# jdfxzzy/DPMN

Measured on AMD Instinct MI355X. Metric: SR images/sec (16x64->32x128, bs=48 per GPU, fp32 forward), higher is better.
Workload: dtype f32; 1 GPU; cfg1: TATT PSN + 3+3 PGRM (embed 96, windows 2/4/8) + CMM, forward-only; per_gpu_batch=48, global_batch=48, ranks=1, batches_in_flight=2, parallelism=dp1 (independent batch shards, no forward collective)

## Files before the change

### dpmn_amd/_abi.py

```python
import ctypes as C
import os

import torch

_HERE = os.path.dirname(os.path.abspath(__file__))
LIB_PATH = os.environ.get("DPMN_HIP_LIB") or os.path.join(_HERE, "lib", "libdpmn_hip.so")

if not os.path.exists(LIB_PATH):
    raise RuntimeError(
        "dpmn_amd: %s not found -- build it with `python -c 'import __graft_entry__ as g; g.build()'` "
        "(or `make -C dpmn_amd/csrc`).  There is no CPU fallback for the DPMN hot path." % LIB_PATH)

lib = C.CDLL(LIB_PATH)

fp = C.c_void_p


class PgrmBlock(C.Structure):
    _fields_ = [(n, fp) for n in (
        "norm1_q_w", "norm1_q_b", "norm1_kv_w", "norm1_kv_b", "q_w", "q_b", "kv_w", "kv_b")] + [
        ("bias_table", fp * 4)] + [(n, fp) for n in (
            "sk_proj_w", "sk_proj_b", "sk_fc1_w", "sk_fc1_b", "sk_fc2_w", "sk_fc2_b", "sk_head_w", "sk_head_b",
            "norm2_w", "norm2_b", "fc1_w", "fc1_b", "dw_w", "dw_b", "pw_w", "pw_b", "fc2_w", "fc2_b")]

# ... 118 lines not shown
    "dpmn_distill_forward_f32": (_i, [C.POINTER(DistillParams), fp, fp, _i, fp, fp, fp, fp, fp, _sz, _i, _i, _i, fp]),
    "dpmn_distill_backward_f32": (_i, [C.POINTER(DistillParams), C.POINTER(DistillGrads), fp, fp, fp, fp, fp, fp, fp, fp, fp, _sz, _i, _i, _i, fp]),
    "dpmn_conv2d_wgrad_unpack_multi_f32": (_i, [fp, fp, _i, _i, fp]),
    "dpmn_tl_interp_f32": (_i, [fp, fp, _i, _i, _i, _i, _i, fp]),
    "dpmn_pointwise_wgrad_det_bytes": (_sz, [_i, _i]),
    "dpmn_reduce_defer_begin": (_i, []),
    "dpmn_reduce_defer_enable": (_i, [_i]),
    "dpmn_reduce_defer_push": (_i, [C.POINTER(TnPending)]),
    "dpmn_reduce_defer_pending": (_i, []),
    "dpmn_reduce_defer_flush": (_i, [_i, fp]),
    "dpmn_xred_fallbacks": (_i, [C.POINTER(C.c_uint), _i]),
    "dpmn_selftest_xshfl": (_i, [C.POINTER(C.c_uint)]),
    "dpmn_selftest_lds_poison": (_i, [C.c_uint, _i, fp]),
    "dpmn_xred_test_force_recompute": (_i, [_i]),
    "dpmn_xred_enable": (_i, [_i]),
    "dpmn_nchw_to_nhwc_f32": (_i, [fp, fp, _i, _i, _i, _i, _i, fp]),
    "dpmn_nhwc_to_nchw_f32": (_i, [fp, fp, _i, _i, _i, _i, fp]),
    "dpmn_se_gate_f32": (_i, [fp, fp, fp, fp, fp, fp, fp, _i, _i, _i, _i, fp]),
    "dpmn_bigru_f32": (_i, [fp, fp, fp, fp, fp, _i, _i, _i, C.c_long, C.c_long, C.c_long, _i, fp]),
    "dpmn_small_linear_f32": (_i, [fp, fp, _i, fp, fp, fp, _i, _i, _i, _i, _f, fp]),
    "dpmn_tatt_encoder_layer_f32": (_i, [fp, fp, _PP, fp, _i, _i, _i, _i, fp]),
    "dpmn_cross_attn_f32": (_i, [fp, fp, fp, fp, fp, _i, _i, _i, _i, _i, fp]),
    "dpmn_add_layernorm64_f32": (_i, [fp, fp, fp, fp, fp, fp, fp, fp, _f, _i, C.c_long, fp]),
    "dpmn_gru_gate_f32": (_i, [fp, fp, fp, fp, C.c_long, _i, _i, fp]),
    "dpmn_to_mask_f32": (_i, [fp, C.c_long, fp, _i, _i, _i, fp]),
    "dpmn_mha32_f32": (_i, [fp, fp, _i, _i, _i, _f, fp]),
    "dpmn_layernorm_std_f32": (_i, [fp, fp, fp, _f, fp, _l, _i, fp]),
    "dpmn_rotate_img_f32": (_i, [fp, fp, fp, _f, fp, _i, _i, _i, _i, fp]),
    "dpmn_blend_f32": (_i, [fp, C.c_long, fp, C.c_long, fp, _f, _i, _i, fp]),
    "dpmn_psnr_ssim_workspace_bytes": (_sz, [_i, _i, _i, _i]),
# ... 227 lines not shown
```

### dpmn_amd/csrc/conv.hip

```cpp
#include "conv_body.h"

namespace {

template <int BM, int BN, int WM, int WN, bool UNI = false, bool SIMPLE = false, bool AFF = false, bool BF = false>
__global__ __launch_bounds__(256) void k_conv_igemm(ConvArgs a) {
  conv_igemm_body<BM, BN, WM, WN, UNI, SIMPLE, AFF, BF>(a);
}
template <int BM, int BN, int WM, int WN, bool AFF>
__global__ __launch_bounds__(256, 2) void k_conv_igemm_xr(ConvArgs a) {
  conv_igemm_body<BM, BN, WM, WN, true, true, AFF, false, true>(a);
}

__global__ __launch_bounds__(256) void k_conv_splitk_reduce(ConvArgs a, int rows, int cq_lanes) {
  __shared__ float red[256][8];
  const PhaseSel ph = conv_select_phase(a, blockIdx.z * a.ksplit);
  const int M = a.B * a.Hp * a.Wp;
  const int n4 = a.npad / 4;
  const int cl = threadIdx.x & (cq_lanes - 1), rl = threadIdx.x / cq_lanes, RL = 256 / cq_lanes;
  const int cq = blockIdx.x * cq_lanes + cl;
  const int n = cq * 4;
  const int m_lo = blockIdx.y * rows;
  float ssum[4] = {0.f, 0.f, 0.f, 0.f}, ssq[4] = {0.f, 0.f, 0.f, 0.f};
  const size_t zs = (size_t)M * a.npad;
  if (cq < n4) {
// ... 704 lines not shown
  for (int i = 0; i < 3; ++i)
    uni = uni && a.cseg[i] % 32 == 0 && (size_t)a.B * a.Hin * a.Win * a.cseg[i] * 4 < (1ull << 31);
  {
    ProfScope prof(BN == 128 ? PT_CONV_IGEMM_128 : (BN == 64 ? PT_CONV_IGEMM_64 : PT_CONV_IGEMM_NARROW), st, conv_flops(a), conv_bytes(a));
    static const int xred_env = getenv("DPMN_CONV_XRED") ? atoi(getenv("DPMN_CONV_XRED")) : 0;
    const int xred_on = g_xred_enabled >= 0 ? g_xred_enabled : xred_env;
    bool simple = uni && a.KH * a.KW <= 31 && (a.pro_act == ACT_NONE || a.pro_act == ACT_RELU || a.pro_act == ACT_LEAKY02);
    int n_seg = 0, n_aff = 0;
    for (int i = 0; i < 3; ++i) {
      if (a.cseg[i] > 0) { ++n_seg; n_aff += a.in_scale[i] != nullptr; }
      simple = simple &&
               ((size_t)a.B * a.Hin * a.Win + (size_t)(abs(a.pad_y) + a.KH * abs(a.dil_y) + 2) * a.Win) * a.cseg[i] * 4 < (1ull << 31);
    }
    simple = simple && (n_aff == 0 || n_aff == n_seg);
  if (g_dpmn_x3 && simple && BM == 128 && BN == 128) {
    if (dpmn_conv::x3_launch_igemm(n_aff != 0, a, grid, st) != 0) return dpmn_set_error(DPMN_ERR_LAUNCH, "conv2d: bf16x3 launch failed");
  } else
  if (g_dpmn_bf16 && simple && BM == BN && (BM == 128 || BM == 64)) {
    if (n_aff) hipLaunchKernelGGL((k_conv_igemm<BM, BN, WM, WN, true, true, true, true>), grid, dim3(256), 0, st, a);
    else hipLaunchKernelGGL((k_conv_igemm<BM, BN, WM, WN, true, true, false, true>), grid, dim3(256), 0, st, a);
  } else
  if (simple && S > 1 && BM == 128 && BN == 128 && xred_on && cnt && xred_fits(tiles, S, cnt_len, a) &&
           (size_t)tiles * S * BM * BN * sizeof(float) <= ws_bytes) {
    if constexpr (BM == 128 && BN == 128) {
      const int tm = cdiv(M, BM), tn = cdiv(a.Cout, BN), t8 = cdiv(tiles, 8);
      double cost[2];
      for (int order = 0; order < 2; ++order) {
        double wsets = 0, xsets = 0;
        for (int c = 0; c < 8; ++c) {
          const int t0 = c * t8, t1 = (c + 1) * t8 < tiles ? (c + 1) * t8 : tiles;
          if (t0 >= t1) break;
// ... 9 lines not shown
          }
        }
        cost[order] = wsets * BN * (double)a.Kp + xsets * BM * (double)a.stride * a.stride * a.cin;
      }
      static const int force_order = getenv("DPMN_XRED_ORDER") ? atoi(getenv("DPMN_XRED_ORDER")) : -1;
      static const int ablate = getenv("DPMN_XRED_ABLATE") ? atoi(getenv("DPMN_XRED_ABLATE")) : 0;
      a.xr_cnt = cnt; a.xr_tm = tm; a.xr_tn = tn; a.xr_t8 = t8; a.xr_force_redo = g_xred_force_recompute; a.xr_ablate = ablate;
      a.xr_order = force_order >= 0 ? force_order : (cost[0] <= cost[1] ? 0 : 1);
      a.wlocal = 0;
      const dim3 g1(8 * t8 * S);
      if (n_aff) hipLaunchKernelGGL((k_conv_igemm_xr<BM, BN, WM, WN, true>), g1, dim3(256), 0, st, a);
      else hipLaunchKernelGGL((k_conv_igemm_xr<BM, BN, WM, WN, false>), g1, dim3(256), 0, st, a);
      DPMN_CHECK_LAUNCH();
      return DPMN_OK;
    }
  }
  else if (simple && n_aff) hipLaunchKernelGGL((k_conv_igemm<BM, BN, WM, WN, true, true, true>), grid, dim3(256), 0, st, a);
  else if (simple) hipLaunchKernelGGL((k_conv_igemm<BM, BN, WM, WN, true, true>), grid, dim3(256), 0, st, a);
  else if (uni) hipLaunchKernelGGL((k_conv_igemm<BM, BN, WM, WN, true>), grid, dim3(256), 0, st, a);
    else hipLaunchKernelGGL((k_conv_igemm<BM, BN, WM, WN>), grid, dim3(256), 0, st, a);
  }
  DPMN_CHECK_LAUNCH();
  if (S > 1) {
    ProfScope prof(PT_CONV_SPLITK_REDUCE, st, 0.0, 4.0 * (double)(S + 1) * nph * M * a.npad);
    const int n4 = a.npad / 4;
    const int cql = n4 >= 64 ? 64 : (n4 >= 32 ? 32 : 16);
    const int cb = cdiv(n4, cql);
    int rows = cb * cdiv(M, 64) >= 1024 ? 64 : (cb * cdiv(M, 16) >= 1024 ? 16 : 4);
    if (rows < 256 / cql) rows = 256 / cql;
    hipLaunchKernelGGL(k_conv_splitk_reduce, dim3(cb, cdiv(M, rows), nph), dim3(256), 0, st, a, rows, cql);
// ... 115 lines not shown
  unsigned v = 0;
  if (hipMemcpyFromSymbol(&v, HIP_SYMBOL(g_xred_fallbacks), sizeof(v)) != hipSuccess) return dpmn_set_error(DPMN_ERR_RUNTIME, "xred_fallbacks: copy failed");
  *count_out = v;
  if (reset) {
    v = 0;
    if (hipMemcpyToSymbol(HIP_SYMBOL(g_xred_fallbacks), &v, sizeof(v)) != hipSuccess) return dpmn_set_error(DPMN_ERR_RUNTIME, "xred_fallbacks: reset failed");
  }
  return DPMN_OK;
}

int dpmn_xred_enable(int on) {
  g_xred_enabled = on < 0 ? -1 : (on ? 1 : 0);
  return DPMN_OK;
}

int dpmn_xred_test_force_recompute(int on) {
  g_xred_force_recompute = on ? 1 : 0;
  return DPMN_OK;
}

int dpmn_nchw_to_nhwc_f32(const float* in, float* out, int B, int C, int H, int W, int Cpad, dpmn_stream_t stream) {
  DPMN_REQUIRE(in && out && Cpad >= C, "nchw_to_nhwc: bad arguments");
  const long total = (long)B * H * W;
  hipLaunchKernelGGL(k_nchw_to_nhwc, dim3((unsigned)((total + 255) / 256)), dim3(256), 0, as_stream(stream), in, out, B, C, H, W, Cpad);
  DPMN_CHECK_LAUNCH();
  return DPMN_OK;
}

int dpmn_nhwc_to_nchw_f32(const float* in, float* out, int B, int C, int H, int W, dpmn_stream_t stream) {
  DPMN_REQUIRE(in && out, "nhwc_to_nchw: bad arguments");
// ... 8 lines not shown
```

### dpmn_amd/csrc/conv_body.h

```cpp
#pragma once
#include <cstdlib>
#include <type_traits>
#include "common.h"

namespace dpmn_conv {
struct ConvArgs {
  const float* in[3];
  const float* in_scale[3];
  const float* in_shift[3];
  int cseg[3];
  int cin;
  int B, Hin, Win;
  int KH, KW, stride, dil_y, dil_x, pad_y, pad_x;
  int Hp, Wp;
  int Hout, Wout, ostep, ooy, oox;
  int pro_act;
  const float* w;
  int Kp;
  const float* bias;
  int Cout;
  int epi_act;
  float slope;
  const float* res;
  float* out;
// ... 6 lines not shown
  int npad;
  int nphase;
  long wps;
  int groups;
  int m_per_group;
  long wgs;
  int wlocal;
  unsigned* xr_cnt;
  int xr_tm, xr_tn;
  int xr_t8;
  int xr_order;
  int xr_force_redo;
  int xr_group;
  int xr_cstride;
  int xr_ablate;
};
int x3_launch_igemm(bool aff, const ConvArgs& a, dim3 grid, hipStream_t st);
int x3_launch_halo(const ConvArgs& a, dim3 grid, hipStream_t st);
}

namespace {

constexpr int PAD = 4, BK = 32, LDK = BK + PAD;
constexpr int STAT_SLOTS = 32;

using dpmn_conv::ConvArgs;
int g_xred_enabled = -1;
int g_xred_force_recompute = 0;
__device__ unsigned g_xred_fallbacks = 0;
__device__ __forceinline__ int conv_group_of(const ConvArgs& a, int m) { return (a.groups > 1 && m >= a.m_per_group) ? 1 : 0; }

struct PhaseSel {
// ... 57 lines not shown
        if (n + r < a.Cout) {
          const float t = v[r] + (a.res ? a.res[o + r] : 0.f);
          a.out[o + r] = post ? fmaxf(t, 0.f) : t;
        }
    }
  }
}

__device__ __forceinline__ float vmax_raw(float x, float y) {
  float r;
  asm("v_max_f32 %0, %1, %2" : "=v"(r) : "v"(x), "v"(y));
  return r;
}

template <int BM, int BN, int WM, int WN, bool UNI = false, bool SIMPLE = false, bool AFF = false, bool BF = false, bool XRED = false,
          bool X3 = false>
__device__ __forceinline__ void conv_igemm_body(const ConvArgs& a) {
  static_assert(!X3 || (SIMPLE && !BF && !XRED), "the bf16x3 variant exists for the SIMPLE path");
  static_assert(!XRED || SIMPLE, "the in-L2 reduction exists for the SIMPLE path");
  static_assert(!BF || SIMPLE, "the bf16 variant exists for the SIMPLE path");
  static_assert(!SIMPLE || UNI, "SIMPLE is a refinement of the UNI path");
  static_assert(!AFF || SIMPLE, "AFF is a variant of the SIMPLE path");
  constexpr int MT = BM / WM / 16, NT = BN / WN / 16;
  constexpr int TPR = BK / 4, RPP = 256 / TPR;
  constexpr int APASS = BM / RPP, BPASS = (BN + RPP - 1) / RPP;
  constexpr int LDKB = X3 ? BK + 16 : BK + 8;
  constexpr bool B16 = BF || X3;
  constexpr int NPL = X3 ? 3 : 1;
  constexpr int NBUF = X3 ? 1 : 2;
  constexpr int XPL = BM * LDKB, WPL = BN * LDKB;
  typedef typename std::conditional<B16, unsigned short, float>::type lds_t;
  __shared__ __attribute__((aligned(16))) lds_t Xs[NBUF][NPL * BM * (B16 ? LDKB : LDK)];
// ... 1 lines not shown

  const int tid = threadIdx.x, lane = tid & 63, wave = tid >> 6;
  const int M = a.B * a.Hp * a.Wp;
  int bx = blockIdx.x, by = blockIdx.y, bz = blockIdx.z;
  int xr_tile = 0;
  if constexpr (XRED) {
    const int L = blockIdx.x, c = L & 7, j = L >> 3;
    const int tl = j / a.ksplit, z = j - tl * a.ksplit;
    const int nph_ = a.nphase > 1 ? a.nphase : 1;
    xr_tile = c * a.xr_t8 + tl;
    if (tl >= a.xr_t8 || xr_tile >= a.xr_tm * a.xr_tn * nph_) return;
    int phs;
    if (a.xr_order == 0) { bx = xr_tile % a.xr_tm; const int r = xr_tile / a.xr_tm; by = r % a.xr_tn; phs = r / a.xr_tn; }
    else { by = xr_tile % a.xr_tn; const int r = xr_tile / a.xr_tn; phs = r % nph_; bx = r / nph_; }
    bz = phs * a.ksplit + z;
  } else
  if (a.wlocal) {
    const int L = bx + gridDim.x * (by + gridDim.y * bz);
    const int c = L & 7, j = L >> 3;
    const int jm = j / (int)gridDim.x;
    bx = j - jm * (int)gridDim.x;
    const int nz = c + 8 * jm;
    by = nz / (int)gridDim.z;
    bz = nz - by * (int)gridDim.z;
  }
  const int m_blk = bx * BM, n_blk = by * BN;
  const PhaseSel ph = conv_select_phase(a, bz, m_blk);
  const int zsplit = ph.zsplit;
  const int lrow = tid / TPR, lcol = (tid % TPR) * 4;

  int pb[APASS], py[APASS], px[APASS];
  const int HWp = a.Hp * a.Wp;
  const float inv_hw = 1.0f / (float)HWp, inv_w = 1.0f / (float)a.Wp;
#pragma unroll
  for (int p = 0; p < APASS; ++p) {
    const int m = m_blk + lrow + p * RPP;
    if (m < M) {
      int b = (int)((float)m * inv_hw), r = m - b * HWp;
      if (r < 0) { --b; r += HWp; }
      if (r >= HWp) { ++b; r -= HWp; }
      int y = (int)((float)r * inv_w), x = r - y * a.Wp;
      if (x < 0) { --y; x += a.Wp; }
      if (x >= a.Wp) { ++y; x -= a.Wp; }
      pb[p] = b;
      py[p] = y * a.stride - ph.pad_y;
      px[p] = x * a.stride - ph.pad_x;
    } else {
      pb[p] = -1; py[p] = 0; px[p] = 0;
    }
  }
  const int c01 = a.cseg[0] + a.cseg[1];
  const int ktaps = a.KH * a.KW;

  float4 xr[APASS], wr[BPASS];
  float4 s4r, h4r;
  unsigned vmask = 0;
  bool has_aff = false;
  auto gload = [&](int k0) {
    const int k = k0 + lcol;
    const int tap = k / a.cin, c = k - tap * a.cin;
    const int ky = tap / a.KW, kx = tap - ky * a.KW;
    const int dy = ky * a.dil_y, dx = kx * a.dil_x;
    int seg = 0, cl = c;
    if (c >= c01) { seg = 2; cl = c - c01; }
    else if (c >= a.cseg[0]) { seg = 1; cl = c - a.cseg[0]; }
// ... 10 lines not shown
      const int iy = py[p] + dy, ix = px[p] + dx;
      const bool ok = pb[p] >= 0 && tap_ok && iy >= 0 && iy < a.Hin && ix >= 0 && ix < a.Win;
      xr[p] = ok ? *reinterpret_cast<const float4*>(src + (((size_t)pb[p] * a.Hin + iy) * a.Win + ix) * cs + cl)
                 : make_float4(0.f, 0.f, 0.f, 0.f);
      vmask |= (ok ? 1u : 0u) << p;
    }
#pragma unroll
    for (int p = 0; p < BPASS; ++p) {
      const int r = lrow + p * RPP;
      const int n = n_blk + r;
      wr[p] = (r < BN && n < a.Cout) ? *reinterpret_cast<const float4*>(ph.w + (size_t)n * a.Kp + k0 + lcol)
                                     : make_float4(0.f, 0.f, 0.f, 0.f);
    }
  };
  typedef int i32x4_ __attribute__((ext_vector_type(4)));
  int pix[APASS];
#pragma unroll
  for (int p = 0; p < APASS; ++p) {
    pix[p] = pb[p] >= 0 ? (pb[p] * a.Hin + py[p]) * a.Win + px[p] : 0;
    if (pb[p] < 0) { py[p] = -(1 << 20); px[p] = -(1 << 20); }
  }
  int u_tap = 0, u_c0 = 0, u_ky = 0, u_kx = 0, u_k0 = -2;
  int wofs[BPASS];
#pragma unroll
  for (int p = 0; p < BPASS; ++p) wofs[p] = ((n_blk + lrow + p * RPP) * a.Kp + lcol) * 4;
  auto gload_uni = [&](int k0) {
    if (k0 == u_k0 + BK) {
      u_c0 += BK;
      if (u_c0 >= a.cin) { u_c0 = 0; ++u_tap; if (++u_kx == a.KW) { u_kx = 0; ++u_ky; } }
    } else if (k0 != u_k0) {
      u_tap = k0 / a.cin; u_c0 = k0 - u_tap * a.cin;
      u_ky = u_tap / a.KW; u_kx = u_tap - u_ky * a.KW;
    }
    u_k0 = k0;
    const int tap = u_tap, c0 = u_c0, ky = u_ky, kx = u_kx;
    const bool tap_ok = tap < ktaps;
    const int dy = tap_ok ? ky * a.dil_y : (1 << 21), dx = kx * a.dil_x;
    const int seg = c0 >= c01 ? 2 : (c0 >= a.cseg[0] ? 1 : 0);
    const int cl = c0 - (seg == 2 ? c01 : (seg == 1 ? a.cseg[0] : 0)) + lcol;
    const float* src = a.in[seg];
// ... 8 lines not shown
    vmask = 0;
#pragma unroll
    for (int p = 0; p < APASS; ++p) {
      const bool ok = (unsigned)(py[p] + dy) < (unsigned)a.Hin && (unsigned)(px[p] + dx) < (unsigned)a.Win;
      const unsigned off = (unsigned)((__mul24(pix[p] + tapoff, cs) + cl) * 4) | (ok ? 0u : 0x80000000u);
      xr[p] = __builtin_bit_cast(float4, __builtin_amdgcn_raw_buffer_load_b128(xrs, (int)off, 0, 0));
      vmask |= (ok ? 1u : 0u) << p;
    }
#pragma unroll
    for (int p = 0; p < BPASS; ++p) {
      const int r = lrow + p * RPP;
      if (BN % RPP == 0 || r < BN)
        wr[p] = __builtin_bit_cast(float4, __builtin_amdgcn_raw_buffer_load_b128(wrs, wofs[p], k0 * 4, 0));
    }
  };
  unsigned nok[APASS];
  int voff[APASS];
  int s_seg = -1, s_segstart = 0;
  __amdgpu_buffer_rsrc_t s_xrs, s_scrs, s_shrs;
  unsigned inv[APASS];
  const int padoff = ph.pad_y * a.Win + ph.pad_x;
  const int minoff = (a.dil_y < 0 ? (a.KH - 1) * a.dil_y : 0) * a.Win + (a.dil_x < 0 ? (a.KW - 1) * a.dil_x : 0);
  const int baseshift = padoff - minoff;
  if (SIMPLE) {
#pragma unroll
    for (int p = 0; p < APASS; ++p) {
      unsigned colm = 0, okb = 0;
      for (int kx = 0; kx < a.KW; ++kx) colm |= ((unsigned)(px[p] + kx * a.dil_x) < (unsigned)a.Win ? 1u : 0u) << kx;
      for (int ky = 0; ky < a.KH; ++ky)
        if ((unsigned)(py[p] + ky * a.dil_y) < (unsigned)a.Hin) okb |= colm << (ky * a.KW);
      nok[p] = ~okb;
    }
  }
  const __amdgpu_buffer_rsrc_t s_wrs = __builtin_amdgcn_make_buffer_rsrc(const_cast<float*>(ph.w), 0, a.Cout * a.Kp * 4, 0x00020000);
  auto gload_simple = [&](int kt_) {
    if (kt_ == u_k0 + 1) {
      ++u_tap;
      if (++u_kx == a.KW) { u_kx = 0; ++u_ky; }
      if (u_tap == ktaps) { u_tap = 0; u_ky = 0; u_c0 += BK; }
    } else if (kt_ != u_k0) {
      const int cch = kt_ / ktaps;
      u_tap = kt_ - cch * ktaps; u_c0 = cch * BK;
      u_ky = u_tap / a.KW; u_kx = u_tap - u_ky * a.KW;
    }
    u_k0 = kt_;
    const int k0 = u_tap * a.cin + u_c0;
    const int seg = u_c0 >= c01 ? 2 : (u_c0 >= a.cseg[0] ? 1 : 0);
    const int cs = seg == 2 ? a.cseg[2] : (seg == 1 ? a.cseg[1] : a.cseg[0]);
    if (seg != s_seg) {
// ... 99 lines not shown
      } else if ((vmask >> p) & 1u) {
        if (has_aff) { v.x = v.x * s4r.x + h4r.x; v.y = v.y * s4r.y + h4r.y; v.z = v.z * s4r.z + h4r.z; v.w = v.w * s4r.w + h4r.w; }
        if (a.pro_act != ACT_NONE) {
          v.x = apply_act(v.x, a.pro_act, 0.f); v.y = apply_act(v.y, a.pro_act, 0.f);
          v.z = apply_act(v.z, a.pro_act, 0.f); v.w = apply_act(v.w, a.pro_act, 0.f);
        }
      }
      *reinterpret_cast<float4*>(&Xs[buf][(lrow + p * RPP) * LDK + lcol]) = v;
    }
#pragma unroll
    for (int p = 0; p < BPASS; ++p)
      if (lrow + p * RPP < BN) *reinterpret_cast<float4*>(&Ws[buf][(lrow + p * RPP) * LDK + lcol]) = wr[p];
    }
  };

  const int wm = wave % WM, wn = wave / WM;
  const int lr = lane & 15, kq = lane >> 4;
  f32x4 acc[NT][MT];
#pragma unroll
  for (int i = 0; i < NT; ++i)
#pragma unroll
    for (int j = 0; j < MT; ++j) acc[i][j] = (f32x4){0.f, 0.f, 0.f, 0.f};

  const int nk_all = a.Kp / BK;
  const int cps = (nk_all + a.ksplit - 1) / a.ksplit;
  int zcur = zsplit;
  int mode = 0;
  for (;;) {
  const int kt0 = zcur * cps;
  const int nk = min(nk_all, kt0 + cps);
  if constexpr (XRED) {
#pragma unroll
    for (int i = 0; i < NT; ++i)
#pragma unroll
      for (int j = 0; j < MT; ++j) acc[i][j] = (f32x4){0.f, 0.f, 0.f, 0.f};
  }
  if (kt0 < nk) {
    if (SIMPLE) { gload_simple(kt0); sstore_simple(0); }
    else {
      if (UNI) gload_uni(kt0 * BK); else gload(kt0 * BK);
      sstore(0);
    }
  }
  __syncthreads();
  for (int kt = kt0; kt < nk; ++kt) {
    const int buf = NBUF == 2 ? (kt - kt0) & 1 : 0;
    if (SIMPLE) gload_simple(min(kt + 1, nk - 1));
    else if (UNI) gload_uni(min(kt + 1, nk - 1) * BK);
    else if (kt + 1 < nk) gload((kt + 1) * BK);
    if (UNI) __builtin_amdgcn_sched_barrier(0);
    if constexpr (X3) {
      const lds_t* xa = &Xs[buf][(wm * (MT * 16) + lr) * LDKB + kq * 8];
      const lds_t* wa = &Ws[buf][(wn * (NT * 16) + lr) * LDKB + kq * 8];
      bf16x8 w0[NT], w1[NT], w2[NT], xp[MT], xq[MT];
#pragma unroll
      for (int i = 0; i < NT; ++i) {
        w0[i] = *reinterpret_cast<const bf16x8*>(wa + i * 16 * LDKB);
// ... 36 lines not shown
#pragma unroll
      for (int i = 0; i < NT; ++i) wf[i] = *reinterpret_cast<const f32x4*>(wa + i * 16 * LDK + kc);
#pragma unroll
      for (int s = 0; s < 4; ++s)
#pragma unroll
        for (int i = 0; i < NT; ++i)
#pragma unroll
          for (int j = 0; j < MT; ++j) acc[i][j] = mfma16(wf[i][s], xf[j][s], acc[i][j]);
    }
    }
    if (NBUF == 1) __syncthreads();
    if (SIMPLE) sstore_simple(NBUF == 2 ? buf ^ 1 : 0);
    else if (UNI || kt + 1 < nk) sstore(buf ^ 1);
    __syncthreads();
  }
  if constexpr (!XRED) break;
  else {
    if (a.ksplit <= 1) break;
    constexpr int QN = NT * MT, HQ = QN / 2;
    static_assert(QN % 2 == 0, "the collect moves half slots");
    typedef int i32x4x_ __attribute__((ext_vector_type(4)));
    const int S = a.ksplit, GS = a.xr_group, ngrp = (S + GS - 1) / GS;
    const int g_lo = (zsplit / GS) * GS, g_hi = min(S, g_lo + GS);
    const __amdgpu_buffer_rsrc_t prs = __builtin_amdgcn_make_buffer_rsrc(a.partial, 0, a.xr_tm * a.xr_tn * (a.nphase > 1 ? a.nphase : 1) * S * (QN * 4096), 0x00020000);
    constexpr int SC1 = 0x10;
    auto slot_of = [&](int z_) { return __builtin_amdgcn_readfirstlane((xr_tile * S + z_) * (QN * 4096)); };
    auto st_slot = [&](int z_) {
      const int so = slot_of(z_);
#pragma unroll
      for (int i = 0; i < NT; ++i)
#pragma unroll
// ... 78 lines not shown
        break;
      }
    }
    if (to_l2) {
      if (ngrp == 1) break;
      st_slot(g_lo);
      const int f = arrive(words + ngrp * a.xr_cstride, ngrp);
      if (f == 0) return;
      if (f == 2) { mode = 2; zcur = 0; continue; }
      if (!(a.xr_ablate & 1)) collect(0, ngrp, GS);
    }
    break;
  }
  }

  if (!XRED && a.ksplit > 1) {
#pragma unroll
    for (int j = 0; j < MT; ++j) {
      const int m = m_blk + wm * (MT * 16) + j * 16 + lr;
      if (m >= M) continue;
#pragma unroll
      for (int i = 0; i < NT; ++i) {
        const int n = n_blk + wn * (NT * 16) + i * 16 + kq * 4;
        if (n >= a.npad) continue;
        *reinterpret_cast<float4*>(ph.partial + ((size_t)zsplit * M + m) * a.npad + n) =
            make_float4(acc[i][j][0], acc[i][j][1], acc[i][j][2], acc[i][j][3]);
      }
    }
    return;
  }
  float ssum[NT][4], ssq[NT][4];
#pragma unroll
  for (int i = 0; i < NT; ++i)
#pragma unroll
    for (int r = 0; r < 4; ++r) { ssum[i][r] = 0.f; ssq[i][r] = 0.f; }
#pragma unroll
  for (int j = 0; j < MT; ++j) {
    const int m = m_blk + wm * (MT * 16) + j * 16 + lr;
    if (m >= M) continue;
#pragma unroll
    for (int i = 0; i < NT; ++i) {
      const int n = n_blk + wn * (NT * 16) + i * 16 + kq * 4;
      if (n >= a.Cout) continue;
      float v[4] = {acc[i][j][0], acc[i][j][1], acc[i][j][2], acc[i][j][3]};
      conv_store(a, m, n, v, ssum[i], ssq[i], ph.ooy, ph.oox);
    }
  }
  if (a.stats) {
#pragma unroll
    for (int i = 0; i < NT; ++i) {
      const int n = n_blk + wn * (NT * 16) + i * 16 + kq * 4;
#pragma unroll
      for (int r = 0; r < 4; ++r) {
        float s = ssum[i][r], q = ssq[i][r];
        s += xshfl<1>(s); s += xshfl<2>(s); s += xshfl<4>(s); s += xshfl<8>(s);
        q += xshfl<1>(q); q += xshfl<2>(q); q += xshfl<4>(q); q += xshfl<8>(q);
        if (lr == 0 && n + r < a.Cout) {
          double* st = reinterpret_cast<double*>(a.stats) + (size_t)(bx % STAT_SLOTS) * 2 * a.Cout;
          atomicAdd(st + n + r, (double)(s));
          atomicAdd(st + a.Cout + n + r, (double)(q));
        }
      }
    }
  }
}

template <int KS, int BN, int TH, bool BF = false, bool X3 = false>
__device__ __forceinline__ void conv_halo_body(const ConvArgs& a) {
  static_assert(!(BF && X3), "one operand format");
  constexpr int NTH = 256, RPS = NTH / 8;
  constexpr int LDH = (BF || X3) ? (BK + 8) / 2 : LDK;
  constexpr int NPL = X3 ? 3 : 1;
  constexpr int TW = 16, HH = TH + KS - 1, HW_ = TW + KS - 1, NPX = HH * HW_;
  constexpr int NT = BN / 16, T = KS * KS, MR = TH / 4;
  constexpr int WV = (BN * 8 + NTH - 1) / NTH;
  constexpr int TPS = 1;
  extern __shared__ __attribute__((aligned(16))) float smem[];
  float* halo = smem;
  float* Wt = smem + NPL * NPX * LDH;
// ... 267 lines not shown
```

### dpmn_amd/csrc/conv_x3.hip

```cpp
#include "conv_body.h"

namespace {
template <int BM, int BN, int WM, int WN, bool AFF>
__global__ __launch_bounds__(256, 2) void k_conv_igemm_x3(ConvArgs a) {
  conv_igemm_body<BM, BN, WM, WN, true, true, AFF, false, false, true>(a);
}
}

namespace dpmn_conv {
int x3_launch_igemm(bool aff, const ConvArgs& a, dim3 grid, hipStream_t st) {
  if (aff) hipLaunchKernelGGL((k_conv_igemm_x3<128, 128, 2, 2, true>), grid, dim3(256), 0, st, a);
  else hipLaunchKernelGGL((k_conv_igemm_x3<128, 128, 2, 2, false>), grid, dim3(256), 0, st, a);
  return 0;
}
int x3_launch_halo(const ConvArgs& a, dim3 grid, hipStream_t st) {
  constexpr int NPX = (8 + 2) * (16 + 2);
  const size_t smem = (size_t)(3 * NPX + 2 * 3 * 64) * ((BK + 8) / 2) * sizeof(float);
  static bool attr_set = false;
  if (!attr_set) {
    (void)hipFuncSetAttribute(reinterpret_cast<const void*>(&k_conv_halo_x3<3, 64, 8>), hipFuncAttributeMaxDynamicSharedMemorySize, (int)smem);
    attr_set = true;
  }
  hipLaunchKernelGGL((k_conv_halo_x3<3, 64, 8>), grid, dim3(256), smem, st, a);
  return 0;
}
}
```

### include/dpmn_hip.h

```cpp
#ifndef DPMN_HIP_H
#define DPMN_HIP_H

#include <stddef.h>
#include <stdint.h>

#ifdef __cplusplus
extern "C" {
#endif

typedef void* dpmn_stream_t;

enum { DPMN_OK = 0, DPMN_ERR_ARG = -1, DPMN_ERR_LAUNCH = -2, DPMN_ERR_WORKSPACE = -3, DPMN_ERR_RUNTIME = -4 };

enum { DPMN_ACT_NONE = 0, DPMN_ACT_GELU = 1, DPMN_ACT_RELU = 2, DPMN_ACT_LEAKY02 = 3, DPMN_ACT_LEAKY001 = 4,
       DPMN_ACT_MISH = 5, DPMN_ACT_PRELU = 6, DPMN_ACT_TANH = 7, DPMN_ACT_SIGMOID = 8,
       DPMN_ACT_RELU_POST_RES = 9  };

int dpmn_abi_version(void);
const char* dpmn_last_error(void);
int dpmn_set_compute_dtype(int mode);
int dpmn_get_compute_dtype(void);

int dpmn_linear_f32(const float* x, const float* w, const float* bias, const float* res1, const float* res2,
                    float* y, int M, int N, int K, int act, float slope, dpmn_stream_t stream);
// ... 84 lines not shown
  float* stats;
  float* splitk_ws;
  size_t splitk_ws_bytes;
  int nphase;
  long w_phase_stride;
  int groups;
  long w_group_stride;
  unsigned* arrive_cnt;
  int arrive_cnt_len;
} dpmn_conv_desc;
int dpmn_conv2d_nhwc_f32(const dpmn_conv_desc* d, dpmn_stream_t stream);
int dpmn_xred_fallbacks(unsigned* count_out, int reset);
int dpmn_selftest_xshfl(unsigned* mismatches_out);
int dpmn_selftest_lds_poison(unsigned pattern, int blocks, dpmn_stream_t stream);
int dpmn_xred_enable(int on);
int dpmn_xred_test_force_recompute(int on);
int dpmn_nchw_to_nhwc_f32(const float* in, float* out, int B, int C, int H, int W, int Cpad, dpmn_stream_t stream);
int dpmn_nhwc_to_nchw_f32(const float* in, float* out, int B, int C, int H, int W, dpmn_stream_t stream);

typedef struct {
  const float *conv_cat_w, *conv_cat_b;
  const float *bn1_w, *bn1_b;
  float *bn1_rm, *bn1_rv;
  long long* bn1_nbt;
  const float *conv_feat_w, *conv_feat_b;
  const float *bn2_w, *bn2_b;
  float *bn2_rm, *bn2_rv;
  long long* bn2_nbt;
} dpmn_distill_params;
typedef struct {
// ... 394 lines not shown
```

Baseline: 6319 images/s.

## Make implicit-GEMM conv kernels persistent with next-tile prefetch overlapping epilogue

Turns the square-tile implicit-GEMM conv kernels, including the bf16x3 variant, into persistent kernels. Each launch sizes its grid to device capacity (CU count times occupancy), and every block loops over output tiles. Before running the current tile's epilogue, a block decodes the next tile and issues its first global fetch, so loads overlap the stores. This is meant to cut wave-tail and launch-granularity costs on small conv grids, at the price of extra register pressure, changed launch bounds, and serialized tiles when there are fewer units than capacity.

New measurement: 6342 images/s (median of 6 runs). No clear change (+0.4%).

```diff
diff --git a/dpmn_amd/_abi.py b/dpmn_amd/_abi.py
--- a/dpmn_amd/_abi.py
+++ b/dpmn_amd/_abi.py
@@ -156,6 +156,7 @@
     "dpmn_selftest_lds_poison": (_i, [C.c_uint, _i, fp]),
     "dpmn_xred_test_force_recompute": (_i, [_i]),
     "dpmn_xred_enable": (_i, [_i]),
+    "dpmn_conv_persist_blocks": (_i, [_i]),
     "dpmn_nchw_to_nhwc_f32": (_i, [fp, fp, _i, _i, _i, _i, _i, fp]),
     "dpmn_nhwc_to_nchw_f32": (_i, [fp, fp, _i, _i, _i, _i, fp]),
     "dpmn_se_gate_f32": (_i, [fp, fp, fp, fp, fp, fp, fp, _i, _i, _i, _i, fp]),
diff --git a/dpmn_amd/csrc/conv.hip b/dpmn_amd/csrc/conv.hip
--- a/dpmn_amd/csrc/conv.hip
+++ b/dpmn_amd/csrc/conv.hip
@@ -6,6 +6,11 @@
 __global__ __launch_bounds__(256) void k_conv_igemm(ConvArgs a) {
   conv_igemm_body<BM, BN, WM, WN, UNI, SIMPLE, AFF, BF>(a);
 }
+template <int BM, int BN, int WM, int WN, bool UNI = false, bool SIMPLE = false, bool AFF = false>
+__global__ __launch_bounds__(256, BM == 64 ? 4 : 2) void k_conv_igemm_p(ConvArgs a) {
+  conv_igemm_body<BM, BN, WM, WN, UNI, SIMPLE, AFF, false, false, false, true>(a);
+}
+int g_persist_blocks = 0;
 template <int BM, int BN, int WM, int WN, bool AFF>
 __global__ __launch_bounds__(256, 2) void k_conv_igemm_xr(ConvArgs a) {
   conv_igemm_body<BM, BN, WM, WN, true, true, AFF, false, true>(a);
@@ -742,7 +747,7 @@
     }
     simple = simple && (n_aff == 0 || n_aff == n_seg);
   if (g_dpmn_x3 && simple && BM == 128 && BN == 128) {
-    if (dpmn_conv::x3_launch_igemm(n_aff != 0, a, grid, st) != 0) return dpmn_set_error(DPMN_ERR_LAUNCH, "conv2d: bf16x3 launch failed");
+    if (dpmn_conv::x3_launch_igemm(n_aff != 0, a, grid, g_persist_blocks, st) != 0) return dpmn_set_error(DPMN_ERR_LAUNCH, "conv2d: bf16x3 launch failed");
   } else
   if (g_dpmn_bf16 && simple && BM == BN && (BM == 128 || BM == 64)) {
     if (n_aff) hipLaunchKernelGGL((k_conv_igemm<BM, BN, WM, WN, true, true, true, true>), grid, dim3(256), 0, st, a);
@@ -782,6 +787,12 @@
       DPMN_CHECK_LAUNCH();
       return DPMN_OK;
     }
+  }
+  else if constexpr (BM == BN) {
+    if (simple && n_aff) launch_conv_units<k_conv_igemm_p<BM, BN, WM, WN, true, true, true>>(a, grid, g_persist_blocks, st);
+    else if (simple) launch_conv_units<k_conv_igemm_p<BM, BN, WM, WN, true, true>>(a, grid, g_persist_blocks, st);
+    else if (uni) launch_conv_units<k_conv_igemm_p<BM, BN, WM, WN, true>>(a, grid, g_persist_blocks, st);
+    else launch_conv_units<k_conv_igemm_p<BM, BN, WM, WN>>(a, grid, g_persist_blocks, st);
   }
   else if (simple && n_aff) hipLaunchKernelGGL((k_conv_igemm<BM, BN, WM, WN, true, true, true>), grid, dim3(256), 0, st, a);
   else if (simple) hipLaunchKernelGGL((k_conv_igemm<BM, BN, WM, WN, true, true>), grid, dim3(256), 0, st, a);
@@ -927,6 +938,12 @@
   return DPMN_OK;
 }
 
+int dpmn_conv_persist_blocks(int n) {
+  const int old = g_persist_blocks;
+  g_persist_blocks = n < 0 ? -1 : n;
+  return old;
+}
+
 int dpmn_xred_test_force_recompute(int on) {
   g_xred_force_recompute = on ? 1 : 0;
   return DPMN_OK;
diff --git a/dpmn_amd/csrc/conv_body.h b/dpmn_amd/csrc/conv_body.h
--- a/dpmn_amd/csrc/conv_body.h
+++ b/dpmn_amd/csrc/conv_body.h
@@ -44,8 +44,10 @@
   int xr_group;
   int xr_cstride;
   int xr_ablate;
+  int p_units;
+  int p_gx, p_gy, p_gz;
 };
-int x3_launch_igemm(bool aff, const ConvArgs& a, dim3 grid, hipStream_t st);
+int x3_launch_igemm(bool aff, const ConvArgs& a, dim3 grid, int blocks, hipStream_t st);
 int x3_launch_halo(const ConvArgs& a, dim3 grid, hipStream_t st);
 }
 
@@ -133,8 +135,9 @@
 }
 
 template <int BM, int BN, int WM, int WN, bool UNI = false, bool SIMPLE = false, bool AFF = false, bool BF = false, bool XRED = false,
-          bool X3 = false>
+          bool X3 = false, bool PERSIST = false>
 __device__ __forceinline__ void conv_igemm_body(const ConvArgs& a) {
+  static_assert(!PERSIST || !XRED, "the in-L2 reduction keeps its own block-to-tile map");
   static_assert(!X3 || (SIMPLE && !BF && !XRED), "the bf16x3 variant exists for the SIMPLE path");
   static_assert(!XRED || SIMPLE, "the in-L2 reduction exists for the SIMPLE path");
   static_assert(!BF || SIMPLE, "the bf16 variant exists for the SIMPLE path");
@@ -166,41 +169,95 @@
     if (a.xr_order == 0) { bx = xr_tile % a.xr_tm; const int r = xr_tile / a.xr_tm; by = r % a.xr_tn; phs = r / a.xr_tn; }
     else { by = xr_tile % a.xr_tn; const int r = xr_tile / a.xr_tn; phs = r % nph_; bx = r / nph_; }
     bz = phs * a.ksplit + z;
-  } else
-  if (a.wlocal) {
-    const int L = bx + gridDim.x * (by + gridDim.y * bz);
-    const int c = L & 7, j = L >> 3;
-    const int jm = j / (int)gridDim.x;
-    bx = j - jm * (int)gridDim.x;
-    const int nz = c + 8 * jm;
-    by = nz / (int)gridDim.z;
-    bz = nz - by * (int)gridDim.z;
-  }
-  const int m_blk = bx * BM, n_blk = by * BN;
-  const PhaseSel ph = conv_select_phase(a, bz, m_blk);
-  const int zsplit = ph.zsplit;
-  const int lrow = tid / TPR, lcol = (tid % TPR) * 4;
-
+  }
+  int m_blk = 0, n_blk = 0, zsplit = 0;
+  PhaseSel ph{};
+  const int lrow0 = tid / TPR, lcol0 = (tid % TPR) * 4;
+  const int lrow = lrow0, lcol = lcol0;
   int pb[APASS], py[APASS], px[APASS];
   const int HWp = a.Hp * a.Wp;
   const float inv_hw = 1.0f / (float)HWp, inv_w = 1.0f / (float)a.Wp;
-#pragma unroll
-  for (int p = 0; p < APASS; ++p) {
-    const int m = m_blk + lrow + p * RPP;
-    if (m < M) {
-      int b = (int)((float)m * inv_hw), r = m - b * HWp;
-      if (r < 0) { --b; r += HWp; }
-      if (r >= HWp) { ++b; r -= HWp; }
-      int y = (int)((float)r * inv_w), x = r - y * a.Wp;
-      if (x < 0) { --y; x += a.Wp; }
-      if (x >= a.Wp) { ++y; x -= a.Wp; }
-      pb[p] = b;
-      py[p] = y * a.stride - ph.pad_y;
-      px[p] = x * a.stride - ph.pad_x;
-    } else {
-      pb[p] = -1; py[p] = 0; px[p] = 0;
-    }
-  }
+  int pix[APASS];
+  int u_tap = 0, u_c0 = 0, u_ky = 0, u_kx = 0, u_k0 = -2;
+  int wofs[BPASS];
+  unsigned nok[APASS];
+  int s_seg = -1;
+  int padoff = 0, baseshift = 0;
+  const int minoff = (a.dil_y < 0 ? (a.KH - 1) * a.dil_y : 0) * a.Win + (a.dil_x < 0 ? (a.KW - 1) * a.dil_x : 0);
+  __amdgpu_buffer_rsrc_t s_wrs;
+  auto unit_decode = [&](int L) {
+    int lrow = lrow0, lcol = lcol0;
+    if constexpr (PERSIST) {
+      asm volatile("" : "+v"(lrow), "+v"(lcol));
+      const int gx = a.p_gx, gy = a.p_gy, gz = a.p_gz;
+      if (a.wlocal) {
+        const int c = L & 7, j = L >> 3;
+        const int jm = j / gx;
+        bx = j - jm * gx;
+        const int nz = c + 8 * jm;
+        by = nz / gz;
+        bz = nz - by * gz;
+      } else {
+        const int r = L / gx;
+        bx = L - r * gx;
+        bz = r / gy;
+        by = r - bz * gy;
+      }
+    } else if constexpr (!XRED) {
+      if (a.wlocal) {
+        const int L_ = bx + gridDim.x * (by + gridDim.y * bz);
+        const int c = L_ & 7, j = L_ >> 3;
+        const int jm = j / (int)gridDim.x;
+        bx = j - jm * (int)gridDim.x;
+        const int nz = c + 8 * jm;
+        by = nz / (int)gridDim.z;
+        bz = nz - by * (int)gridDim.z;
+      }
+    }
+    m_blk = bx * BM; n_blk = by * BN;
+    ph = conv_select_phase(a, bz, m_blk);
+    zsplit = ph.zsplit;
+#pragma unroll
+    for (int p = 0; p < APASS; ++p) {
+      const int m = m_blk + lrow + p * RPP;
+      if (m < M) {
+        int b = (int)((float)m * inv_hw), r = m - b * HWp;
+        if (r < 0) { --b; r += HWp; }
+        if (r >= HWp) { ++b; r -= HWp; }
+        int y = (int)((float)r * inv_w), x = r - y * a.Wp;
+        if (x < 0) { --y; x += a.Wp; }
+        if (x >= a.Wp) { ++y; x -= a.Wp; }
+        pb[p] = b;
+        py[p] = y * a.stride - ph.pad_y;
+        px[p] = x * a.stride - ph.pad_x;
+      } else {
+        pb[p] = -1; py[p] = 0; px[p] = 0;
+      }
+    }
+#pragma unroll
+    for (int p = 0; p < APASS; ++p) {
+      pix[p] = pb[p] >= 0 ? (pb[p] * a.Hin + py[p]) * a.Win + px[p] : 0;
+      if (pb[p] < 0) { py[p] = -(1 << 20); px[p] = -(1 << 20); }
+    }
+    u_k0 = -2; s_seg = -1;
+#pragma unroll
+    for (int p = 0; p < BPASS; ++p) wofs[p] = ((n_blk + lrow + p * RPP) * a.Kp + lcol) * 4;
+    padoff = ph.pad_y * a.Win + ph.pad_x;
+    baseshift = padoff - minoff;
+    if (SIMPLE) {
+#pragma unroll
+      for (int p = 0; p < APASS; ++p) {
+        unsigned colm = 0, okb = 0;
+        for (int kx = 0; kx < a.KW; ++kx) colm |= ((unsigned)(px[p] + kx * a.dil_x) < (unsigned)a.Win ? 1u : 0u) << kx;
+        for (int ky = 0; ky < a.KH; ++ky)
+          if ((unsigned)(py[p] + ky * a.dil_y) < (unsigned)a.Hin) okb |= colm << (ky * a.KW);
+        nok[p] = ~okb;
+      }
+    }
+    s_wrs = __builtin_amdgcn_make_buffer_rsrc(const_cast<float*>(ph.w), 0, a.Cout * a.Kp * 4, 0x00020000);
+  };
+  int unit = PERSIST ? (int)blockIdx.x : 0;
+  unit_decode(unit);
   const int c01 = a.cseg[0] + a.cseg[1];
   const int ktaps = a.KH * a.KW;
 
@@ -241,16 +298,6 @@
     }
   };
   typedef int i32x4_ __attribute__((ext_vector_type(4)));
-  int pix[APASS];
-#pragma unroll
-  for (int p = 0; p < APASS; ++p) {
-    pix[p] = pb[p] >= 0 ? (pb[p] * a.Hin + py[p]) * a.Win + px[p] : 0;
-    if (pb[p] < 0) { py[p] = -(1 << 20); px[p] = -(1 << 20); }
-  }
-  int u_tap = 0, u_c0 = 0, u_ky = 0, u_kx = 0, u_k0 = -2;
-  int wofs[BPASS];
-#pragma unroll
-  for (int p = 0; p < BPASS; ++p) wofs[p] = ((n_blk + lrow + p * RPP) * a.Kp + lcol) * 4;
   auto gload_uni = [&](int k0) {
     if (k0 == u_k0 + BK) {
       u_c0 += BK;
@@ -289,25 +336,10 @@
         wr[p] = __builtin_bit_cast(float4, __builtin_amdgcn_raw_buffer_load_b128(wrs, wofs[p], k0 * 4, 0));
     }
   };
-  unsigned nok[APASS];
   int voff[APASS];
-  int s_seg = -1, s_segstart = 0;
+  int s_segstart = 0;
   __amdgpu_buffer_rsrc_t s_xrs, s_scrs, s_shrs;
   unsigned inv[APASS];
-  const int padoff = ph.pad_y * a.Win + ph.pad_x;
-  const int minoff = (a.dil_y < 0 ? (a.KH - 1) * a.dil_y : 0) * a.Win + (a.dil_x < 0 ? (a.KW - 1) * a.dil_x : 0);
-  const int baseshift = padoff - minoff;
-  if (SIMPLE) {
-#pragma unroll
-    for (int p = 0; p < APASS; ++p) {
-      unsigned colm = 0, okb = 0;
-      for (int kx = 0; kx < a.KW; ++kx) colm |= ((unsigned)(px[p] + kx * a.dil_x) < (unsigned)a.Win ? 1u : 0u) << kx;
-      for (int ky = 0; ky < a.KH; ++ky)
-        if ((unsigned)(py[p] + ky * a.dil_y) < (unsigned)a.Hin) okb |= colm << (ky * a.KW);
-      nok[p] = ~okb;
-    }
-  }
-  const __amdgpu_buffer_rsrc_t s_wrs = __builtin_amdgcn_make_buffer_rsrc(const_cast<float*>(ph.w), 0, a.Cout * a.Kp * 4, 0x00020000);
   auto gload_simple = [&](int kt_) {
     if (kt_ == u_k0 + 1) {
       ++u_tap;
@@ -437,8 +469,9 @@
     }
   };
 
-  const int wm = wave % WM, wn = wave / WM;
-  const int lr = lane & 15, kq = lane >> 4;
+  const int wm0 = wave % WM, wn0 = wave / WM;
+  const int lr0 = lane & 15, kq0 = lane >> 4;
+  const int wm = wm0, wn = wn0, lr = lr0, kq = kq0;
   f32x4 acc[NT][MT];
 #pragma unroll
   for (int i = 0; i < NT; ++i)
@@ -449,6 +482,68 @@
   const int cps = (nk_all + a.ksplit - 1) / a.ksplit;
   int zcur = zsplit;
   int mode = 0;
+  auto first_fetch = [&](int z_) {
+    const int k_ = z_ * cps;
+    if (k_ < nk_all) {
+      if (SIMPLE) gload_simple(k_);
+      else if (UNI) gload_uni(k_ * BK);
+      else gload(k_ * BK);
+    }
+  };
+  auto epilogue = [&](int m_blk_, int n_blk_, int bx_, int z_, int ooy_, int oox_, float* partial_) {
+    int wm = wm0, wn = wn0, lr = lr0, kq = kq0;
+    if constexpr (PERSIST) asm volatile("" : "+v"(wm), "+v"(wn), "+v"(lr), "+v"(kq));
+    if (!XRED && a.ksplit > 1) {
+#pragma unroll
+      for (int j = 0; j < MT; ++j) {
+        const int m = m_blk_ + wm * (MT * 16) + j * 16 + lr;
+        if (m >= M) continue;
+#pragma unroll
+        for (int i = 0; i < NT; ++i) {
+          const int n = n_blk_ + wn * (NT * 16) + i * 16 + kq * 4;
+          if (n >= a.npad) continue;
+          *reinterpret_cast<float4*>(partial_ + ((size_t)z_ * M + m) * a.npad + n) =
+              make_float4(acc[i][j][0], acc[i][j][1], acc[i][j][2], acc[i][j][3]);
+        }
+      }
+      return;
+    }
+    float ssum[NT][4], ssq[NT][4];
+#pragma unroll
+    for (int i = 0; i < NT; ++i)
+#pragma unroll
+      for (int r = 0; r < 4; ++r) { ssum[i][r] = 0.f; ssq[i][r] = 0.f; }
+#pragma unroll
+    for (int j = 0; j < MT; ++j) {
+      const int m = m_blk_ + wm * (MT * 16) + j * 16 + lr;
+      if (m >= M) continue;
+#pragma unroll
+      for (int i = 0; i < NT; ++i) {
+        const int n = n_blk_ + wn * (NT * 16) + i * 16 + kq * 4;
+        if (n >= a.Cout) continue;
+        float v[4] = {acc[i][j][0], acc[i][j][1], acc[i][j][2], acc[i][j][3]};
+        conv_store(a, m, n, v, ssum[i], ssq[i], ooy_, oox_);
+      }
+    }
+    if (a.stats) {
+#pragma unroll
+      for (int i = 0; i < NT; ++i) {
+        const int n = n_blk_ + wn * (NT * 16) + i * 16 + kq * 4;
+#pragma unroll
+        for (int r = 0; r < 4; ++r) {
+          float s = ssum[i][r], q = ssq[i][r];
+          s += xshfl<1>(s); s += xshfl<2>(s); s += xshfl<4>(s); s += xshfl<8>(s);
+          q += xshfl<1>(q); q += xshfl<2>(q); q += xshfl<4>(q); q += xshfl<8>(q);
+          if (lr == 0 && n + r < a.Cout) {
+            double* st = reinterpret_cast<double*>(a.stats) + (size_t)(bx_ % STAT_SLOTS) * 2 * a.Cout;
+            atomicAdd(st + n + r, (double)(s));
+            atomicAdd(st + a.Cout + n + r, (double)(q));
+          }
+        }
+      }
+    }
+  };
+  if constexpr (PERSIST) first_fetch(zsplit);
   for (;;) {
   const int kt0 = zcur * cps;
   const int nk = min(nk_all, kt0 + cps);
@@ -458,12 +553,9 @@
 #pragma unroll
       for (int j = 0; j < MT; ++j) acc[i][j] = (f32x4){0.f, 0.f, 0.f, 0.f};
   }
+  if constexpr (!PERSIST) first_fetch(zcur);
   if (kt0 < nk) {
-    if (SIMPLE) { gload_simple(kt0); sstore_simple(0); }
-    else {
-      if (UNI) gload_uni(kt0 * BK); else gload(kt0 * BK);
-      sstore(0);
-    }
+    if (SIMPLE) sstore_simple(0); else sstore(0);
   }
   __syncthreads();
   for (int kt = kt0; kt < nk; ++kt) {
@@ -530,7 +622,24 @@
     else if (UNI || kt + 1 < nk) sstore(buf ^ 1);
     __syncthreads();
   }
-  if constexpr (!XRED) break;
+  if constexpr (PERSIST) {
+    const int e_m = m_blk, e_n = n_blk, e_bx = bx, e_z = zsplit, e_ooy = ph.ooy, e_oox = ph.oox;
+    float* const e_partial = ph.partial;
+    unit += (int)gridDim.x;
+    const bool more = unit < a.p_units;
+    if (more) {
+      unit_decode(unit);
+      zcur = zsplit;
+      first_fetch(zsplit);
+      __builtin_amdgcn_sched_barrier(0);
+    }
+    epilogue(e_m, e_n, e_bx, e_z, e_ooy, e_oox, e_partial);
+    if (!more) return;
+#pragma unroll
+    for (int i = 0; i < NT; ++i)
+#pragma unroll
+      for (int j = 0; j < MT; ++j) acc[i][j] = (f32x4){0.f, 0.f, 0.f, 0.f};
+  } else if constexpr (!XRED) break;
   else {
     if (a.ksplit <= 1) break;
     constexpr int QN = NT * MT, HQ = QN / 2;
@@ -639,55 +748,25 @@
   }
   }
 
-  if (!XRED && a.ksplit > 1) {
-#pragma unroll
-    for (int j = 0; j < MT; ++j) {
-      const int m = m_blk + wm * (MT * 16) + j * 16 + lr;
-      if (m >= M) continue;
-#pragma unroll
-      for (int i = 0; i < NT; ++i) {
-        const int n = n_blk + wn * (NT * 16) + i * 16 + kq * 4;
-        if (n >= a.npad) continue;
-        *reinterpret_cast<float4*>(ph.partial + ((size_t)zsplit * M + m) * a.npad + n) =
-            make_float4(acc[i][j][0], acc[i][j][1], acc[i][j][2], acc[i][j][3]);
-      }
-    }
-    return;
-  }
-  float ssum[NT][4], ssq[NT][4];
-#pragma unroll
-  for (int i = 0; i < NT; ++i)
-#pragma unroll
-    for (int r = 0; r < 4; ++r) { ssum[i][r] = 0.f; ssq[i][r] = 0.f; }
-#pragma unroll
-  for (int j = 0; j < MT; ++j) {
-    const int m = m_blk + wm * (MT * 16) + j * 16 + lr;
-    if (m >= M) continue;
-#pragma unroll
-    for (int i = 0; i < NT; ++i) {
-      const int n = n_blk + wn * (NT * 16) + i * 16 + kq * 4;
-      if (n >= a.Cout) continue;
-      float v[4] = {acc[i][j][0], acc[i][j][1], acc[i][j][2], acc[i][j][3]};
-      conv_store(a, m, n, v, ssum[i], ssq[i], ph.ooy, ph.oox);
-    }
-  }
-  if (a.stats) {
-#pragma unroll
-    for (int i = 0; i < NT; ++i) {
-      const int n = n_blk + wn * (NT * 16) + i * 16 + kq * 4;
-#pragma unroll
-      for (int r = 0; r < 4; ++r) {
-        float s = ssum[i][r], q = ssq[i][r];
-        s += xshfl<1>(s); s += xshfl<2>(s); s += xshfl<4>(s); s += xshfl<8>(s);
-        q += xshfl<1>(q); q += xshfl<2>(q); q += xshfl<4>(q); q += xshfl<8>(q);
-        if (lr == 0 && n + r < a.Cout) {
-          double* st = reinterpret_cast<double*>(a.stats) + (size_t)(bx % STAT_SLOTS) * 2 * a.Cout;
-          atomicAdd(st + n + r, (double)(s));
-          atomicAdd(st + a.Cout + n + r, (double)(q));
-        }
-      }
-    }
-  }
+  epilogue(m_blk, n_blk, bx, zsplit, ph.ooy, ph.oox, ph.partial);
+}
+
+template <void (*KERN)(ConvArgs)>
+void launch_conv_units(ConvArgs a, dim3 grid, int blocks, hipStream_t st) {
+  static int capacity = 0;
+  if (!capacity) {
+    int dev = 0, cus = 0, per_cu = 0;
+    (void)hipGetDevice(&dev);
+    (void)hipDeviceGetAttribute(&cus, hipDeviceAttributeMultiprocessorCount, dev);
+    (void)hipOccupancyMaxActiveBlocksPerMultiprocessor(&per_cu, reinterpret_cast<const void*>(KERN), 256, 0);
+    capacity = (cus > 0 ? cus : 256) * (per_cu > 0 ? per_cu : 2);
+    if (capacity >= 8) capacity &= ~7;
+  }
+  const long units = (long)grid.x * grid.y * grid.z;
+  a.p_gx = (int)grid.x; a.p_gy = (int)grid.y; a.p_gz = (int)grid.z; a.p_units = (int)units;
+  long G = blocks > 0 ? blocks : (blocks < 0 ? units : capacity);
+  if (G > units) G = units;
+  hipLaunchKernelGGL(KERN, dim3((unsigned)G), dim3(256), 0, st, a);
 }
 
 template <int KS, int BN, int TH, bool BF = false, bool X3 = false>
diff --git a/dpmn_amd/csrc/conv_x3.hip b/dpmn_amd/csrc/conv_x3.hip
--- a/dpmn_amd/csrc/conv_x3.hip
+++ b/dpmn_amd/csrc/conv_x3.hip
@@ -3,14 +3,14 @@
 namespace {
 template <int BM, int BN, int WM, int WN, bool AFF>
 __global__ __launch_bounds__(256, 2) void k_conv_igemm_x3(ConvArgs a) {
-  conv_igemm_body<BM, BN, WM, WN, true, true, AFF, false, false, true>(a);
+  conv_igemm_body<BM, BN, WM, WN, true, true, AFF, false, false, true, true>(a);
 }
 }
 
 namespace dpmn_conv {
-int x3_launch_igemm(bool aff, const ConvArgs& a, dim3 grid, hipStream_t st) {
-  if (aff) hipLaunchKernelGGL((k_conv_igemm_x3<128, 128, 2, 2, true>), grid, dim3(256), 0, st, a);
-  else hipLaunchKernelGGL((k_conv_igemm_x3<128, 128, 2, 2, false>), grid, dim3(256), 0, st, a);
+int x3_launch_igemm(bool aff, const ConvArgs& a, dim3 grid, int blocks, hipStream_t st) {
+  if (aff) launch_conv_units<k_conv_igemm_x3<128, 128, 2, 2, true>>(a, grid, blocks, st);
+  else launch_conv_units<k_conv_igemm_x3<128, 128, 2, 2, false>>(a, grid, blocks, st);
   return 0;
 }
 int x3_launch_halo(const ConvArgs& a, dim3 grid, hipStream_t st) {
diff --git a/include/dpmn_hip.h b/include/dpmn_hip.h
--- a/include/dpmn_hip.h
+++ b/include/dpmn_hip.h
@@ -122,6 +122,7 @@
 int dpmn_selftest_xshfl(unsigned* mismatches_out);
 int dpmn_selftest_lds_poison(unsigned pattern, int blocks, dpmn_stream_t stream);
 int dpmn_xred_enable(int on);
+int dpmn_conv_persist_blocks(int n);
 int dpmn_xred_test_force_recompute(int on);
 int dpmn_nchw_to_nhwc_f32(const float* in, float* out, int B, int C, int H, int W, int Cpad, dpmn_stream_t stream);
 int dpmn_nhwc_to_nchw_f32(const float* in, float* out, int B, int C, int H, int W, dpmn_stream_t stream);
```
